# oleg-savchenko/jax_nbody_emulator_with_dj

Measured on AMD Instinct MI355X. Metric: voxels/sec (disp+vel) on 512^3 box, ndiv=4, higher is better.
Workload: dtype f32-equivalent: f16x3 split MFMA (3 f16 MFMAs per product, f32 accumulate)

## Files before the change

jax_nbody_emulator_with_dj_amd/csrc/nbe_kernels_h3.hip:

```cpp

#include "nbe_kernels_internal.h"
#include <cstdlib>
#include <cstdio>
#include <algorithm>

#ifndef NBE_DBG
#define NBE_DBG 0
#endif

namespace nbe {

extern __shared__ __attribute__((aligned(16))) f32x4 lds_h3[];

__device__ __forceinline__ void split4(const f32x4 v, half4& hi, half4& lo) {
#pragma unroll
    for (int e = 0; e < 4; ++e) {
        hi[e] = (_Float16)v[e];
        lo[e] = (_Float16)__builtin_fmaf((float)hi[e], -H3_SCALE, v[e] * H3_SCALE);
    }
}
__device__ __forceinline__ f32x4 join4(const half4 hi, const half4 lo) {
    f32x4 v;
#pragma unroll
    for (int e = 0; e < 4; ++e) v[e] = (float)hi[e] + (float)lo[e] * H3_INV;
    return v;
}

template <bool VEL, bool SPLIT>
__device__ __forceinline__ void h3_store2(const ConvKArgs& a, int ct, int it, int lh, const long (&o)[2],
                                          const bool (&ok)[2], const f32x16 (&ym)[2], const f32x16 (&yc)[2],
                                          const f32x16 (&dm)[2], const f32x16 (&dc)[2]) {
    constexpr int PARTS = SPLIT ? 2 : 1;
    const bool act = a.flags & F_ACT, res = a.flags & F_RES;
    int unit[4];
    bool uok[4];
    f32x4 bv[4], gv[4];
    const bool gauge = VEL && a.gout;
#pragma unroll
    for (int k = 0; k < 4; ++k) {
        unit[k] = ct * 8 + 4 * it + k;
        uok[k] = unit[k] < a.cout_groups;
        if (!uok[k]) unit[k] = a.cout_groups - 1;
        bv[k] = *(const f32x4*)(a.bias + unit[k] * 8 + 4 * lh);
        if (gauge) gv[k] = *(const f32x4*)(a.gout + unit[k] * 8 + 4 * lh);
    }
    half4 rh[8], rl[8], dh[8], dl[8];
    if (res) {
#pragma unroll
        for (int p = 0; p < 8; ++p) {
            const long rb = ((long)(PARTS * unit[p & 3]) * a.res_pstride + o[p >> 2]) * 16 + 8 * lh;
            const long rlo = rb + a.res_pstride * 16;
            rh[p] = *(const half4*)((const char*)a.r + rb);
            if (SPLIT) rl[p] = *(const half4*)((const char*)a.r + rlo);
            if (VEL) {
                dh[p] = *(const half4*)((const char*)a.dr + rb);
                if (SPLIT) dl[p] = *(const half4*)((const char*)a.dr + rlo);
            }
        }
    }
#pragma unroll
    for (int p = 0; p < 8; ++p) {
        const int jt = p >> 2, k = p & 3;
        f32x4 v, dv;
#pragma unroll
        for (int e = 0; e < 4; ++e) {
            v[e] = ym[jt][4 * k + e] + (SPLIT ? yc[jt][4 * k + e] * H3_INV : 0.f) + bv[k][e];
            dv[e] = dm[jt][4 * k + e] + (SPLIT ? dc[jt][4 * k + e] * H3_INV : 0.f);
        }
        if (res) {
            if (SPLIT) {
                v += join4(rh[p], rl[p]);
                if (VEL) dv += join4(dh[p], dl[p]);
            } else {
#pragma unroll
                for (int e = 0; e < 4; ++e) {
                    v[e] += (float)rh[p][e];
                    if (VEL) dv[e] += (float)dh[p][e];
                }
            }
        }
        if (act) {
#pragma unroll
            for (int e = 0; e < 4; ++e) {
                if (VEL) dv[e] = v[e] > 0.f ? dv[e] : 0.01f * dv[e];
                v[e] = v[e] >= 0.f ? v[e] : 0.01f * v[e];
            }
        }
        if (gauge) {
#pragma unroll
            for (int e = 0; e < 4; ++e) dv[e] += gv[k][e] * v[e];
        }
        if (uok[k] && ok[jt]) {
            const long ob = ((long)(a.out_g0 + PARTS * unit[k]) * a.out_pstride + o[jt]) * 16 + 8 * lh;
            const long ol = ob + a.out_pstride * 16;
            half4 hi, lo;
            split4(v, hi, lo);
            *(half4*)((char*)a.y + ob) = hi;
            if (SPLIT) *(half4*)((char*)a.y + ol) = lo;
            if (VEL) {
                split4(dv, hi, lo);
                *(half4*)((char*)a.dy + ob) = hi;
                if (SPLIT) *(half4*)((char*)a.dy + ol) = lo;
            }
        }
    }
}


template <int MODE, bool SPLIT>
struct H3Geom {
    static constexpr int PARTS = SPLIT ? 2 : 1, UN = 2 * PARTS;
    static_assert(MODE != MODE_FLAT3, "3x3x3 layers run on the patch kernels");
    static constexpr int XV = 256;
    static constexpr int WP = UN * 64;
    static constexpr int XP = UN * XV;
};

template <int MODE, bool VEL, bool HAS_DX, bool SPLIT>
__global__ __launch_bounds__(512, 2) void conv_h3_kernel(ConvKArgs a) {
    typedef H3Geom<MODE, SPLIT> G;
    constexpr int XV = G::XV, WP = G::WP, XP = G::XP, PARTS = G::PARTS, UN = G::UN;
    constexpr bool DX = VEL && HAS_DX;
    constexpr int WB = WP * (VEL ? 2 : 1);
    constexpr int XB = XP * (DX ? 2 : 1);
    constexpr int OFF_DW = WP, OFF_DXX = XP;
    constexpr int XRING = 2 * WB;
    constexpr int NW_TOT = WB / 64, NX_TOT = (XB + 63) / 64;
    constexpr int NWS = (NW_TOT + 7) / 8, NXS = (NX_TOT + 7) / 8;
    static_assert(WB % 64 == 0, "weight stage must be whole wave-instructions");
    static_assert(XP % 32 == 0, "activation planes must be half-wave multiples");
    static_assert(NWS + NXS <= 9, "more DMA slots per wave than MFMA pairs in one stage");

    f32x4* lds = lds_h3;
    const int tid = threadIdx.x;
    const int lane = tid & 63;
    const int wave = __builtin_amdgcn_readfirstlane(tid >> 6);
    const int li = lane & 31, lh = lane >> 5;
    const int it = wave & 1, jq = wave >> 1;

    const int tile = xcd_tile(blockIdx.x, a.ntiles);
    const int ct = blockIdx.y;
    const long q0 = (long)tile * TILE_VOX;
    const int nstage = mode_nseg(MODE) * a.nchunk;
    const long HW = (long)a.H * a.W;

    int* inbase = (int*)(lds + XRING + 2 * XB);
    if (MODE == MODE_DOWN) {
        if (tid < TILE_VOX) {
            long o = q0 + tid;
            if (o > a.Q - 1) o = a.Q - 1;
            const int hw = a.Hv * a.Wv;
            const int zo = (int)(o / hw), rem = (int)(o - (long)zo * hw);
            const int yo = rem / a.Wv, xo = rem - yo * a.Wv;
            inbase[tid] = (int)((2L * zo * a.H + 2 * yo) * a.W + 2 * xo);
        }
        __syncthreads();
    }

    const char* wsrc[NWS];
    int wdst[NWS];
    const char* xsrc[NXS];
    int xdst[NXS];
#pragma unroll
    for (int t = 0; t < NWS; ++t) {
        const int n = wave + 8 * t;
        wsrc[t] = nullptr; wdst[t] = 0;
        if (n < NW_TOT) {
            const bool d = VEL && n >= WP / 64;
            const int m = n - (d ? WP / 64 : 0);
            wsrc[t] = (const char*)(d ? a.dw : a.w) + ((long)ct * nstage * WP + m * 64 + lane) * 16;
            wdst[t] = (d ? OFF_DW : 0) + m * 64;
        }
    }
#pragma unroll
    for (int t = 0; t < NXS; ++t) {
        const int n = wave + 8 * t;
        xsrc[t] = nullptr; xdst[t] = 0;
        if (n < NX_TOT) {
            const int u = n * 64 + lane;
            const bool tang = DX && u >= XP;
            const int uu = u - (tang ? XP : 0);
            const int pl = uu / XV, vl = uu - pl * XV;
            long v;
            if (MODE == MODE_DOWN) v = (long)inbase[vl];
            else v = q0 + a.in_off + vl;
            xsrc[t] = (const char*)(tang ? a.dx : a.x) + ((long)pl * a.in_pstride + v) * 16;
            xdst[t] = (tang ? OFF_DXX : 0) + uu;
            xdst[t] = __builtin_amdgcn_readfirstlane(xdst[t]);
        }
    }

    auto seg_offset = [&](int s) -> long {
        const int chunk = s / mode_nseg(MODE), seg = s - chunk * mode_nseg(MODE);
        long segoff;
        if (MODE == MODE_DOWN) segoff = (seg >> 2) * HW + ((seg >> 1) & 1) * a.W + (seg & 1);
        else segoff = 0;
        return ((long)chunk * UN * a.in_pstride + segoff) * 16;
    };
    auto dma_w = [&](int t, int s) {
        if (wave + 8 * t < NW_TOT) dma16((const float*)(wsrc[t] + (long)s * WP * 16), lds + (s & 1) * WB + wdst[t]);
    };
    auto dma_x = [&](int t, long xoff, int ring) {
        if (wave + 8 * t < NX_TOT) dma16((const float*)(xsrc[t] + xoff), lds + XRING + ring * XB + xdst[t]);
    };
    auto wait_all = [&]() { asm volatile("s_waitcnt vmcnt(0)" ::: "memory"); };
    auto barrier = [&]() { asm volatile("s_waitcnt lgkmcnt(0)\n\ts_barrier" ::: "memory"); };

    f32x16 ym[2], yc[2], dm[2], dc[2];
#pragma unroll
    for (int jt = 0; jt < 2; ++jt)
#pragma unroll
        for (int e = 0; e < 16; ++e) { ym[jt][e] = 0.f; yc[jt][e] = 0.f; dm[jt][e] = 0.f; dc[jt][e] = 0.f; }

    struct Ops { half8 wh, wl, dwh, dwl, xh[2], xl[2], dxh[2], dxl[2]; };
    auto load_ops = [&](const half8* wb, const half8* xb, Ops& o) {
        const int wo = (PARTS * lh) * 64 + 32 * it + li;
        o.wh = wb[wo];
        if (SPLIT) o.wl = wb[wo + 64];
        if (VEL) { o.dwh = wb[OFF_DW + wo]; if (SPLIT) o.dwl = wb[OFF_DW + wo + 64]; }
#pragma unroll
        for (int jt = 0; jt < 2; ++jt) {
            const int xo = (PARTS * lh) * XV + jq * 64 + 32 * jt + li;
            o.xh[jt] = xb[xo];
            if (SPLIT) o.xl[jt] = xb[xo + XV];
            if (DX) { o.dxh[jt] = xb[OFF_DXX + xo]; if (SPLIT) o.dxl[jt] = xb[OFF_DXX + xo + XV]; }
        }
    };
    auto mfma1 = [&](const Ops& o, int i) {
        const int jt = i / 9, k = i % 9;
        if (k == 0) ym[jt] = __builtin_amdgcn_mfma_f32_32x32x16_f16(o.wh, o.xh[jt], ym[jt], 0, 0, 0);
        if (SPLIT && k == 1) yc[jt] = __builtin_amdgcn_mfma_f32_32x32x16_f16(o.wh, o.xl[jt], yc[jt], 0, 0, 0);
        if (SPLIT && k == 2) yc[jt] = __builtin_amdgcn_mfma_f32_32x32x16_f16(o.wl, o.xh[jt], yc[jt], 0, 0, 0);
        if (VEL) {
            if (k == 3) dm[jt] = __builtin_amdgcn_mfma_f32_32x32x16_f16(o.dwh, o.xh[jt], dm[jt], 0, 0, 0);
            if (SPLIT && k == 4) dc[jt] = __builtin_amdgcn_mfma_f32_32x32x16_f16(o.dwh, o.xl[jt], dc[jt], 0, 0, 0);
            if (SPLIT && k == 5) dc[jt] = __builtin_amdgcn_mfma_f32_32x32x16_f16(o.dwl, o.xh[jt], dc[jt], 0, 0, 0);
        }
        if (DX) {
            if (k == 6) dm[jt] = __builtin_amdgcn_mfma_f32_32x32x16_f16(o.wh, o.dxh[jt], dm[jt], 0, 0, 0);
            if (SPLIT && k == 7) dc[jt] = __builtin_amdgcn_mfma_f32_32x32x16_f16(o.wh, o.dxl[jt], dc[jt], 0, 0, 0);
            if (SPLIT && k == 8) dc[jt] = __builtin_amdgcn_mfma_f32_32x32x16_f16(o.wl, o.dxh[jt], dc[jt], 0, 0, 0);
        }
    };

    {
        const long x0 = seg_offset(0);
#pragma unroll
        for (int t = 0; t < NXS; ++t) dma_x(t, x0, 0);
#pragma unroll
        for (int t = 0; t < NWS; ++t) dma_w(t, 0);
        wait_all();
        barrier();
    }

    int ring = 0;
    for (int s = 0; s < nstage; ++s) {
        const bool pw = s + 1 < nstage, px = s + 1 < nstage;
        const long xoff2 = px ? seg_offset(s + 1) : 0;
        const int ring2 = ring ^ 1;
        const half8* wb = (const half8*)(lds + (s & 1) * WB);
        const half8* xb = (const half8*)(lds + XRING + ring * XB);
        Ops o0, o1;
        load_ops(wb, xb, o0);
        __builtin_amdgcn_sched_barrier(0);
#pragma unroll
        for (int i = 0; i < 18; ++i) {
            mfma1(o0, i);
            if (i & 1) {
                const int t = i >> 1;
                if (t < NWS) { if (pw) dma_w(t, s + 1); }
                else if (t - NWS < NXS) { if (px) dma_x(t - NWS, xoff2, ring2); }
                __builtin_amdgcn_sched_barrier(0);
            }
        }
        __builtin_amdgcn_sched_barrier(0);
        __builtin_amdgcn_sched_barrier(0);
        wait_all();
        barrier();
        ring = ring == 1 ? 0 : ring + 1;
    }

    long o[2];
    bool ok[2];
#pragma unroll
    for (int jt = 0; jt < 2; ++jt) {
        const long q = q0 + jq * 64 + 32 * jt + li;
        ok[jt] = q < a.Q;
        if (MODE == MODE_DOWN) {
            o[jt] = q;
        } else {
            const int z = (int)(q / HW), rem = (int)(q - (long)z * HW);
            const int yy = rem / a.W, xx = rem - yy * a.W;
            ok[jt] = ok[jt] && xx < a.Wv && yy < a.Hv && z < a.Dv;
            o[jt] = ((long)(z * a.osz + a.oz) * a.Ho + (yy * a.osz + a.oy)) * a.Wo + (xx * a.osz + a.ox);
        }
        if (!ok[jt]) o[jt] = 0;
    }
    h3_store2<VEL, SPLIT>(a, ct, it, lh, o, ok, ym, yc, dm, dc);
}

constexpr int UP_XV = 256;
constexpr int UP_MAXCH = 4;
template <bool SPLIT> struct UpGeom {
    static constexpr int UN = SPLIT ? 4 : 2;
    static constexpr int XC = 2 * UN * UP_XV;
    static constexpr int WS = 2 * 2 * UN * 64;
    static constexpr int WBASE = UP_MAXCH * XC;
    static constexpr int LDS_UNITS = WBASE + 2 * WS;
};

template <bool SPLIT, bool VEL = true>
__global__ __launch_bounds__(512, 2) void up_h3_kernel(ConvKArgs a) {
    constexpr int UN = UpGeom<SPLIT>::UN, UP_XC = UpGeom<SPLIT>::XC, UP_WS = UpGeom<SPLIT>::WS, UP_WBASE = UpGeom<SPLIT>::WBASE;
    constexpr int PS = SPLIT ? 2 : 1;
    f32x4* lds = lds_h3;
    const half8* L8 = (const half8*)lds_h3;
    const int tid = threadIdx.x;
    const int lane = tid & 63;
    const int wave = __builtin_amdgcn_readfirstlane(tid >> 6);
    const int li = lane & 31, lh = lane >> 5;
    const int it = wave & 1, jq = wave >> 1;
    const int tile = xcd_tile(blockIdx.x, a.ntiles);
    const int ct = blockIdx.y;
    const long q0 = (long)tile * UP_XV;
    const int nchunk = a.nchunk, nstage = 2 * 4 * nchunk;
    const long HW = (long)a.H * a.W;

    for (int c = 0; c < nchunk; ++c) {
#pragma unroll
        for (int k = 0; k < (VEL ? UN : UN / 2); ++k) {
            const int n = wave + 8 * k;
            const int t = n / (4 * UN), u = (n >> 2) % UN, qd = n & 3;
            const long v = q0 + a.in_off + qd * 64 + lane;
            const char* src = (const char*)(t ? a.dx : a.x) + (((long)c * UN + u) * a.in_pstride + v) * 16;
            dma16((const float*)src, lds + c * UP_XC + (t * UN + u) * UP_XV + qd * 64);
        }
    }
    auto dma_w = [&](int st) {
        const int c = st % nchunk, pp = (st / nchunk) & 3;
#pragma unroll
        for (int k = 0; k < UN / 2; ++k) {
            const int n = wave + 8 * k;
            const int par = n / (2 * UN), d = (n / UN) & 1, m = n % UN;
            if (!VEL && d) continue;
            const char* src = (const char*)(d ? a.dw : a.w) + (long)(2 * pp + par) * a.set_stride +
                              (((long)ct * nchunk + c) * (UN * 64) + m * 64 + lane) * 16;
            dma16((const float*)src, lds + UP_WBASE + (st & 1) * UP_WS + n * 64);
        }
    };
    dma_w(0);
    asm volatile("s_waitcnt vmcnt(0)" ::: "memory");
    __syncthreads();

    f32x16 ym[2], yc[2], dm[2], dc[2];
    auto zero_acc = [&]() {
#pragma unroll
        for (int jt = 0; jt < 2; ++jt)
#pragma unroll
            for (int e = 0; e < 16; ++e) { ym[jt][e] = 0.f; yc[jt][e] = 0.f; dm[jt][e] = 0.f; dc[jt][e] = 0.f; }
    };
    zero_acc();

    for (int st = 0; st < nstage; ++st) {
        const int c = st % nchunk, pp = (st / nchunk) & 3, half = st / (4 * nchunk);
        if (st + 1 < nstage) dma_w(st + 1);
        const half8* wb = L8 + UP_WBASE + (st & 1) * UP_WS;
        const half8* xb = L8 + c * UP_XC;
        const int xo = (PS * lh) * UP_XV + half * 128 + jq * 32 + li;
        const half8 xh = xb[xo];
        half8 dxh = xh, xl = xh, dxl = xh;
        if (VEL) dxh = xb[UN * UP_XV + xo];
        if (SPLIT) { xl = xb[xo + UP_XV]; if (VEL) dxl = xb[UN * UP_XV + xo + UP_XV]; }
#pragma unroll
        for (int jt = 0; jt < 2; ++jt) {
            const int wo = jt * (2 * UN * 64) + (PS * lh) * 64 + 32 * it + li;
            const half8 wh = wb[wo];
            half8 dwh = wh;
            if (VEL) dwh = wb[UN * 64 + wo];
            if (!SPLIT) {
                ym[jt] = __builtin_amdgcn_mfma_f32_32x32x16_f16(wh, xh, ym[jt], 0, 0, 0);
                if (VEL) {
                    dm[jt] = __builtin_amdgcn_mfma_f32_32x32x16_f16(dwh, xh, dm[jt], 0, 0, 0);
                    dm[jt] = __builtin_amdgcn_mfma_f32_32x32x16_f16(wh, dxh, dm[jt], 0, 0, 0);
                }
                continue;
            }
            const half8 wl = wb[wo + 64];
            ym[jt] = __builtin_amdgcn_mfma_f32_32x32x16_f16(wh, xh, ym[jt], 0, 0, 0);
            yc[jt] = __builtin_amdgcn_mfma_f32_32x32x16_f16(wh, xl, yc[jt], 0, 0, 0);
            yc[jt] = __builtin_amdgcn_mfma_f32_32x32x16_f16(wl, xh, yc[jt], 0, 0, 0);
            if (!VEL) continue;
            const half8 dwl = wb[UN * 64 + wo + 64];
            dm[jt] = __builtin_amdgcn_mfma_f32_32x32x16_f16(dwh, xh, dm[jt], 0, 0, 0);
            dc[jt] = __builtin_amdgcn_mfma_f32_32x32x16_f16(dwh, xl, dc[jt], 0, 0, 0);
            dc[jt] = __builtin_amdgcn_mfma_f32_32x32x16_f16(dwl, xh, dc[jt], 0, 0, 0);
            dm[jt] = __builtin_amdgcn_mfma_f32_32x32x16_f16(wh, dxh, dm[jt], 0, 0, 0);
            dc[jt] = __builtin_amdgcn_mfma_f32_32x32x16_f16(wh, dxl, dc[jt], 0, 0, 0);
            dc[jt] = __builtin_amdgcn_mfma_f32_32x32x16_f16(wl, dxh, dc[jt], 0, 0, 0);
        }
        const bool epi = c == nchunk - 1;
        if (epi) {
            asm volatile("s_waitcnt vmcnt(0)" ::: "memory");
            const long q = q0 + half * 128 + jq * 32 + li;
            const int z = (int)(q / HW), rem = (int)(q - (long)z * HW);
            const int yy = rem / a.W, xx = rem - yy * a.W;
            const bool okq = q < a.Q && xx < a.Wv && yy < a.Hv && z < a.Dv;
            const long o0 = okq ? ((long)(2 * z + (pp >> 1)) * a.Ho + (2 * yy + (pp & 1))) * a.Wo + 2 * xx : 0;
            const long o[2] = {o0, o0 + (okq ? 1 : 0)};
            const bool ok[2] = {okq, okq};
            h3_store2<VEL, SPLIT>(a, ct, it, lh, o, ok, ym, yc, dm, dc);
            zero_acc();
            asm volatile("s_waitcnt lgkmcnt(0)\n\ts_barrier" ::: "memory");
        } else {
            asm volatile("s_waitcnt vmcnt(0) lgkmcnt(0)" ::: "memory");
            __syncthreads();
        }
    }
}

template <bool SPLIT, bool VEL = true>
static int launch_up_h3(ConvKArgs ka, int ctiles, hipStream_t s) {
    constexpr size_t smem = (size_t)UpGeom<SPLIT>::LDS_UNITS * 16;
    static_assert(smem <= 160 * 1024, "LDS budget of one CU");
    if (ka.nchunk > UP_MAXCH) return 1;
    ensure_lds_limit((const void*)up_h3_kernel<SPLIT, VEL>, smem);
    dim3 grid(ka.ntiles, ctiles, 1), block(512, 1, 1);
    hipLaunchKernelGGL((up_h3_kernel<SPLIT, VEL>), grid, block, smem, s, ka);
    return 0;
}

constexpr int HP_ROWS = 8, HP_COLS = 32;
constexpr int HP_RS = HP_COLS + 2;
constexpr int HP_PL = (HP_ROWS + 2) * HP_RS;

template <bool VEL, bool HAS_DX, bool SPLIT>
__global__ __launch_bounds__(512, 2) void conv_h3p_kernel(ConvKArgs a) {
    constexpr bool DX = VEL && HAS_DX;
    constexpr int PARTS = SPLIT ? 2 : 1, UN = 2 * PARTS;
    constexpr int HP_XP = UN * HP_PL;
    constexpr int HP_XPP = (HP_XP + 63) / 64 * 64;
    constexpr int WP = 3 * UN * 64;
    constexpr int WB = WP * (VEL ? 2 : 1);
    constexpr int XB = HP_XPP * (DX ? 2 : 1);
    constexpr int OFF_DW = WP, OFF_DXX = HP_XPP;
    constexpr int XBASE = 2 * WB;
    constexpr int NW_TOT = WB / 64, NX_TOT = XB / 64;
    constexpr int NWS = (NW_TOT + 7) / 8;
    constexpr int XPARTS = 3;
    constexpr int NXS = (NX_TOT + 8 * XPARTS - 1) / (8 * XPARTS);
    static_assert(NWS + NXS <= 9 && NXS <= 4, "DMA slots per wave");

    f32x4* lds = lds_h3;
    const int tid = threadIdx.x;
    const int lane = tid & 63;
    const int wave = __builtin_amdgcn_readfirstlane(tid >> 6);
    const int li = lane & 31, lh = lane >> 5;
    const int it = wave & 1, jq = wave >> 1;

    const int tile = xcd_tile(blockIdx.x, a.ntiles);
    const int ct = blockIdx.y;
    const int z = tile % a.Dv, tyx = tile / a.Dv;
    const int ty = tyx / a.tnx, tx = tyx - ty * a.tnx;
    const int y0 = ty * HP_ROWS, x0 = tx * HP_COLS;
    const int nstage = 9 * a.nchunk;

    const char* wsrc[NWS];
    int wdst[NWS];
    const char* xsrc[XPARTS][NXS];
    int xdst[XPARTS][NXS];
    int kx[XPARTS];
#pragma unroll
    for (int t = 0; t < NWS; ++t) {
        const int n = wave + 8 * t;
        wsrc[t] = nullptr; wdst[t] = 0;
        if (n < NW_TOT) {
            const bool d = VEL && n >= WP / 64;
            const int m = n - (d ? WP / 64 : 0);
            wsrc[t] = (const char*)(d ? a.dw : a.w) + ((long)ct * nstage * WP + m * 64 + lane) * 16;
            wdst[t] = (d ? OFF_DW : 0) + m * 64;
        }
    }
#pragma unroll
    for (int p = 0; p < XPARTS; ++p) {
        kx[p] = 0;
#pragma unroll
        for (int t = 0; t < NXS; ++t) {
            const int n = (p * NXS + t) * 8 + wave;
            xsrc[p][t] = nullptr; xdst[p][t] = 0;
            if (n < NX_TOT) {
                ++kx[p];
                const int u = n * 64 + lane;
                const bool tang = DX && u >= HP_XPP;
                int uu = u - (tang ? HP_XPP : 0);
                const int ud = uu;
                if (uu >= HP_XP) uu = HP_XP - 1;
                const int pl = uu / HP_PL, rem = uu - pl * HP_PL;
                const int row = rem / HP_RS, col = rem - row * HP_RS;
                xsrc[p][t] = (const char*)(tang ? a.dx : a.x) + ((long)pl * a.in_pstride + (long)row * a.W + col) * 16;
                xdst[p][t] = __builtin_amdgcn_readfirstlane((tang ? OFF_DXX : 0) + ud);
            }
        }
    }
    auto patch_offset = [&](int g) -> long {
        const int chunk = g / 3, dz = g - chunk * 3;
        return ((long)chunk * UN * a.in_pstride + ((long)(z + dz) * a.H + y0) * a.W + x0) * 16;
    };
    auto dma_w = [&](int t, int s) {
        if (wave + 8 * t < NW_TOT) dma16((const float*)(wsrc[t] + (long)s * WP * 16), lds + (s & 1) * WB + wdst[t]);
    };
    auto dma_x = [&](int p, int t, long xoff, int xb) {
        if ((p * NXS + t) * 8 + wave < NX_TOT) dma16((const float*)(xsrc[p][t] + xoff), lds + XBASE + xb * XB + xdst[p][t]);
    };

    f32x16 ym[2], yc[2], dm[2], dc[2];
#pragma unroll
    for (int jt = 0; jt < 2; ++jt)
#pragma unroll
        for (int e = 0; e < 16; ++e) { ym[jt][e] = 0.f; yc[jt][e] = 0.f; dm[jt][e] = 0.f; dc[jt][e] = 0.f; }

    struct Ops { half8 wh, wl, dwh, dwl, xh[2], xl[2], dxh[2], dxl[2]; };
    auto load_ops = [&](const half8* wb, const half8* xb, int dy, int dx, Ops& o) {
        const int wo = (dx * UN + PARTS * lh) * 64 + 32 * it + li;
        o.wh = wb[wo];
        if (SPLIT) o.wl = wb[wo + 64];
        if (VEL) { o.dwh = wb[OFF_DW + wo]; if (SPLIT) o.dwl = wb[OFF_DW + wo + 64]; }
#pragma unroll
        for (int jt = 0; jt < 2; ++jt) {
            const int xo = (PARTS * lh) * HP_PL + (2 * jq + jt + dy) * HP_RS + li + dx;
            o.xh[jt] = xb[xo];
            if (SPLIT) o.xl[jt] = xb[xo + HP_PL];
            if (DX) { o.dxh[jt] = xb[OFF_DXX + xo]; if (SPLIT) o.dxl[jt] = xb[OFF_DXX + xo + HP_PL]; }
        }
    };
    auto mfma1 = [&](const Ops& o, int i) {
        const int jt = i / 9, k = i % 9;
        if (k == 0) ym[jt] = __builtin_amdgcn_mfma_f32_32x32x16_f16(o.wh, o.xh[jt], ym[jt], 0, 0, 0);
        if (SPLIT && k == 1) yc[jt] = __builtin_amdgcn_mfma_f32_32x32x16_f16(o.wh, o.xl[jt], yc[jt], 0, 0, 0);
        if (SPLIT && k == 2) yc[jt] = __builtin_amdgcn_mfma_f32_32x32x16_f16(o.wl, o.xh[jt], yc[jt], 0, 0, 0);
        if (VEL) {
            if (k == 3) dm[jt] = __builtin_amdgcn_mfma_f32_32x32x16_f16(o.dwh, o.xh[jt], dm[jt], 0, 0, 0);
            if (SPLIT && k == 4) dc[jt] = __builtin_amdgcn_mfma_f32_32x32x16_f16(o.dwh, o.xl[jt], dc[jt], 0, 0, 0);
            if (SPLIT && k == 5) dc[jt] = __builtin_amdgcn_mfma_f32_32x32x16_f16(o.dwl, o.xh[jt], dc[jt], 0, 0, 0);
        }
        if (DX) {
            if (k == 6) dm[jt] = __builtin_amdgcn_mfma_f32_32x32x16_f16(o.wh, o.dxh[jt], dm[jt], 0, 0, 0);
            if (SPLIT && k == 7) dc[jt] = __builtin_amdgcn_mfma_f32_32x32x16_f16(o.wh, o.dxl[jt], dc[jt], 0, 0, 0);
            if (SPLIT && k == 8) dc[jt] = __builtin_amdgcn_mfma_f32_32x32x16_f16(o.wl, o.dxh[jt], dc[jt], 0, 0, 0);
        }
    };
    auto mfma_ops = [&](const Ops& o) {
#pragma unroll
        for (int i = 0; i < 18; ++i) mfma1(o, i);
    };

    {
        const long x0off = patch_offset(0);
#pragma unroll
        for (int p = 0; p < XPARTS; ++p)
#pragma unroll
            for (int t = 0; t < NXS; ++t) dma_x(p, t, x0off, 0);
#pragma unroll
        for (int t = 0; t < NWS; ++t) dma_w(t, 0);
        __syncthreads();
    }

    int g = 0, dy = 0;
    for (int s = 0; s < nstage; ++s) {
        const bool pw = s + 1 < nstage, px = 3 * (g + 1) < nstage;
        const long xoff = px ? patch_offset(g + 1) : 0;
        const half8* wb = (const half8*)(lds + (s & 1) * WB);
        const half8* xb = (const half8*)(lds + XBASE + (g & 1) * XB);
        const int nb = (g + 1) & 1;
        Ops o0, o1;
        load_ops(wb, xb, dy, 0, o0);
        load_ops(wb, xb, dy, 1, o1);
        __builtin_amdgcn_sched_barrier(0);
#pragma unroll
        for (int i = 0; i < 18; ++i) {
            mfma1(o0, i);
            if (i & 1) {
                const int t = i >> 1;
                if (t < NWS) { if (pw) dma_w(t, s + 1); }
                else if (t - NWS < NXS) {
                    if (px) {
                        if (dy == 0) dma_x(0, t - NWS, xoff, nb);
                        else if (dy == 1) dma_x(1, t - NWS, xoff, nb);
                        else dma_x(2, t - NWS, xoff, nb);
                    }
                }
                __builtin_amdgcn_sched_barrier(0);
            }
        }
        __builtin_amdgcn_sched_barrier(0);
        load_ops(wb, xb, dy, 2, o0);
        __builtin_amdgcn_sched_barrier(0);
        mfma_ops(o1);
        __builtin_amdgcn_sched_barrier(0);
        mfma_ops(o0);
        __builtin_amdgcn_sched_barrier(0);
        __syncthreads();
        if (++dy == 3) { dy = 0; ++g; }
    }

    long o[2];
    bool ok[2];
#pragma unroll
    for (int jt = 0; jt < 2; ++jt) {
        const int yy = y0 + 2 * jq + jt, xx = x0 + li;
        ok[jt] = yy < a.Hv && xx < a.Wv;
        o[jt] = ok[jt] ? ((long)z * a.Ho + yy) * a.Wo + xx : (long)z * a.Ho * a.Wo;
    }
    h3_store2<VEL, SPLIT>(a, ct, it, lh, o, ok, ym, yc, dm, dc);
}

constexpr int HQ_TAPU = 4 * 64;
constexpr int HQ_WA = 5 * HQ_TAPU, HQ_WB = 4 * HQ_TAPU;
constexpr int HQ_OFF_B = 2 * HQ_WA;
constexpr int HQ_PP = (HP_PL + 7) / 8 * 8;
constexpr int HQ_XT = 4 * HQ_PP;
constexpr int HQ_XB = 2 * HQ_XT;
constexpr int HQ_XBASE = HQ_OFF_B + 2 * HQ_WB;
constexpr int HQ_LDS_UNITS = HQ_XBASE + 2 * HQ_XB;

__device__ __forceinline__ float acc_read(const float& acc) {
    float v;
    asm volatile("v_accvgpr_read_b32 %0, %1" : "=v"(v) : "a"(acc));
    return v;
}

__device__ __forceinline__ void dma16s(const char* ubase, unsigned voff, f32x4* dst_wave_base) {
    const unsigned long ub = (unsigned long)ubase;
    ubase = (const char*)(((unsigned long)(unsigned)__builtin_amdgcn_readfirstlane((int)(ub >> 32)) << 32) |
                          (unsigned long)(unsigned)__builtin_amdgcn_readfirstlane((int)(unsigned)ub));
    asm volatile("" : "+v"(voff));
    __builtin_amdgcn_global_load_lds((const NBE_GLB_AS void*)(ubase + voff), (NBE_LDS_AS void*)dst_wave_base, 16, 0, 0);
}

__device__ unsigned long long h3q_stamps[16];

void h3q_read_stamps(double* out, hipStream_t s) {
    unsigned long long h[16] = {0};
    (void)hipStreamSynchronize(s);
    (void)hipMemcpyFromSymbol(h, HIP_SYMBOL(h3q_stamps), sizeof h, 0, hipMemcpyDeviceToHost);
    for (int i = 0; i < 16; ++i) out[i] = (double)h[i];
    unsigned long long z[16] = {0};
    (void)hipMemcpyToSymbol(HIP_SYMBOL(h3q_stamps), z, sizeof z, 0, hipMemcpyHostToDevice);
}

__global__ __launch_bounds__(512, 2) void conv_h3q_kernel(ConvKArgs a) {
#if NBE_DBG
    unsigned long long tk0 = __builtin_amdgcn_s_memtime(), tk[8] = {0, 0, 0, 0, 0, 0, 0, 0};
#define NBE_STAMP(i) { const unsigned long long t_ = __builtin_amdgcn_s_memtime(); tk[i] += t_ - tk0; tk0 = t_; }
#define NBE_STAGE_END(i, keep) { NBE_STAMP(i) wait_keep(keep); NBE_STAMP(i + 1) \
                                 asm volatile("s_barrier" ::: "memory"); NBE_STAMP(i + 2) }
#else
#define NBE_STAMP(i)
#define NBE_STAGE_END(i, keep) { wait_keep(keep); asm volatile("s_barrier" ::: "memory"); }
#endif
    f32x4* lds = lds_h3;
    const half8* L8 = (const half8*)lds_h3;
    const int tid = threadIdx.x;
    const int lane = tid & 63;
    const int wave = __builtin_amdgcn_readfirstlane(tid >> 6);
    const int c = lane & 15, q = lane >> 4, kh = q & 1, ks = q >> 1;
    const int it = wave & 1, jq = wave >> 1;

    const int nct = (a.cout_groups + 7) / 8;
    const int vt = xcd_tile(blockIdx.x, a.ntiles * nct);
    const int tile = vt / nct, ct = vt - tile * nct;
    const int z = tile % a.Dv, tyx = tile / a.Dv;
    const int ty = tyx / a.tnx, tx = tyx - ty * a.tnx;
    const int y0 = ty * HP_ROWS, x0 = tx * HP_COLS;
    const int ngroups = 3 * a.nchunk;

    const unsigned lane16 = (unsigned)lane * 16u;
    const long wct = (long)ct * ngroups * 9 * HQ_TAPU;
    auto dma_w = [&](int g, int second, int t) {
        const int per = (second ? HQ_WB : HQ_WA) / 64;
        const int n = wave + 8 * t;
        if (n >= 2 * per) return;
        const int set = n >= per ? 1 : 0, m = n - set * per;
        const long src = wct + (long)g * 9 * HQ_TAPU + (second ? 5 * HQ_TAPU : 0) + m * 64;
        dma16s((const char*)(set ? a.dw : a.w) + src * 16, lane16,
               lds + (second ? HQ_OFF_B : 0) + set * (second ? HQ_WB : HQ_WA) + m * 64);
    };
    unsigned xoff[3];
    bool xval[3];
#pragma unroll
    for (int t = 0; t < 3; ++t) {
        const int k = (wave + 8 * t) % 6;
        const int u = k * 64 + lane;
        xval[t] = u < HP_PL;
        const int uu = xval[t] ? u : HP_PL - 1;
        const int row = uu / HP_RS, col = uu - row * HP_RS;
        xoff[t] = (unsigned)(row * a.W + col) * 16u;
    }
    auto patch_offset = [&](int g) -> long {
        const int chunk = g / 3, dz = g - chunk * 3;
        return ((long)chunk * 4 * a.in_pstride + ((long)(z + dz) * a.H + y0) * a.W + x0) * 16;
    };
    auto dma_x = [&](int tensor, int t, long xo, int buf) {
        const int n = wave + 8 * t, pl = n / 6, k = n - 6 * pl;
        if (xval[t])
            dma16s((const char*)(tensor ? a.dx : a.x) + xo + (long)pl * a.in_pstride * 16, xoff[t],
                   lds + HQ_XBASE + buf * HQ_XB + tensor * HQ_XT + pl * HQ_PP + k * 64);
    };
// ... 1318 lines not shown
```

Measured before the change: 97.63 million.

## Remap up-conv waves to cover all voxels per pass, skipping empty cout passes

```diff
diff --git a/jax_nbody_emulator_with_dj_amd/csrc/nbe_kernels_h3.hip b/jax_nbody_emulator_with_dj_amd/csrc/nbe_kernels_h3.hip
--- a/jax_nbody_emulator_with_dj_amd/csrc/nbe_kernels_h3.hip
+++ b/jax_nbody_emulator_with_dj_amd/csrc/nbe_kernels_h3.hip
@@ -301,10 +301,11 @@
 
 constexpr int UP_XV = 256;
 constexpr int UP_MAXCH = 4;
+constexpr int UP_CT = 32;
 template <bool SPLIT> struct UpGeom {
     static constexpr int UN = SPLIT ? 4 : 2;
     static constexpr int XC = 2 * UN * UP_XV;
-    static constexpr int WS = 2 * 2 * UN * 64;
+    static constexpr int WS = 2 * 2 * UN * UP_CT;
     static constexpr int WBASE = UP_MAXCH * XC;
     static constexpr int LDS_UNITS = WBASE + 2 * WS;
 };
@@ -319,11 +320,10 @@
     const int lane = tid & 63;
     const int wave = __builtin_amdgcn_readfirstlane(tid >> 6);
     const int li = lane & 31, lh = lane >> 5;
-    const int it = wave & 1, jq = wave >> 1;
     const int tile = xcd_tile(blockIdx.x, a.ntiles);
     const int ct = blockIdx.y;
     const long q0 = (long)tile * UP_XV;
-    const int nchunk = a.nchunk, nstage = 2 * 4 * nchunk;
+    const int nchunk = a.nchunk, npass = a.cout_groups - 8 * ct > 4 ? 2 : 1, nstage = npass * 4 * nchunk;
     const long HW = (long)a.H * a.W;
 
     for (int c = 0; c < nchunk; ++c) {
@@ -337,15 +337,15 @@
         }
     }
     auto dma_w = [&](int st) {
-        const int c = st % nchunk, pp = (st / nchunk) & 3;
-#pragma unroll
-        for (int k = 0; k < UN / 2; ++k) {
-            const int n = wave + 8 * k;
-            const int par = n / (2 * UN), d = (n / UN) & 1, m = n % UN;
-            if (!VEL && d) continue;
-            const char* src = (const char*)(d ? a.dw : a.w) + (long)(2 * pp + par) * a.set_stride +
-                              (((long)ct * nchunk + c) * (UN * 64) + m * 64 + lane) * 16;
-            dma16((const float*)src, lds + UP_WBASE + (st & 1) * UP_WS + n * 64);
+        const int c = st % nchunk, pp = (st / nchunk) & 3, it = st / (4 * nchunk);
+        if (wave < 2 * UN) {
+            const int r0 = 2 * wave;
+            const int par = r0 / (2 * UN), d = (r0 / UN) & 1, m = r0 % UN + lh;
+            if (VEL || !d) {
+                const char* src = (const char*)(d ? a.dw : a.w) + (long)(2 * pp + par) * a.set_stride +
+                                  (((long)ct * nchunk + c) * (UN * 64) + m * 64 + UP_CT * it + li) * 16;
+                dma16((const float*)src, lds + UP_WBASE + (st & 1) * UP_WS + wave * 64);
+            }
         }
     };
     dma_w(0);
@@ -362,21 +362,21 @@
     zero_acc();
 
     for (int st = 0; st < nstage; ++st) {
-        const int c = st % nchunk, pp = (st / nchunk) & 3, half = st / (4 * nchunk);
+        const int c = st % nchunk, pp = (st / nchunk) & 3, it = st / (4 * nchunk);
         if (st + 1 < nstage) dma_w(st + 1);
         const half8* wb = L8 + UP_WBASE + (st & 1) * UP_WS;
         const half8* xb = L8 + c * UP_XC;
-        const int xo = (PS * lh) * UP_XV + half * 128 + jq * 32 + li;
+        const int xo = (PS * lh) * UP_XV + wave * 32 + li;
         const half8 xh = xb[xo];
         half8 dxh = xh, xl = xh, dxl = xh;
         if (VEL) dxh = xb[UN * UP_XV + xo];
         if (SPLIT) { xl = xb[xo + UP_XV]; if (VEL) dxl = xb[UN * UP_XV + xo + UP_XV]; }
 #pragma unroll
         for (int jt = 0; jt < 2; ++jt) {
-            const int wo = jt * (2 * UN * 64) + (PS * lh) * 64 + 32 * it + li;
+            const int wo = jt * (2 * UN * UP_CT) + (PS * lh) * UP_CT + li;
             const half8 wh = wb[wo];
             half8 dwh = wh;
-            if (VEL) dwh = wb[UN * 64 + wo];
+            if (VEL) dwh = wb[UN * UP_CT + wo];
             if (!SPLIT) {
                 ym[jt] = __builtin_amdgcn_mfma_f32_32x32x16_f16(wh, xh, ym[jt], 0, 0, 0);
                 if (VEL) {
@@ -385,12 +385,12 @@
                 }
                 continue;
             }
-            const half8 wl = wb[wo + 64];
+            const half8 wl = wb[wo + UP_CT];
             ym[jt] = __builtin_amdgcn_mfma_f32_32x32x16_f16(wh, xh, ym[jt], 0, 0, 0);
             yc[jt] = __builtin_amdgcn_mfma_f32_32x32x16_f16(wh, xl, yc[jt], 0, 0, 0);
             yc[jt] = __builtin_amdgcn_mfma_f32_32x32x16_f16(wl, xh, yc[jt], 0, 0, 0);
             if (!VEL) continue;
-            const half8 dwl = wb[UN * 64 + wo + 64];
+            const half8 dwl = wb[UN * UP_CT + wo + UP_CT];
             dm[jt] = __builtin_amdgcn_mfma_f32_32x32x16_f16(dwh, xh, dm[jt], 0, 0, 0);
             dc[jt] = __builtin_amdgcn_mfma_f32_32x32x16_f16(dwh, xl, dc[jt], 0, 0, 0);
             dc[jt] = __builtin_amdgcn_mfma_f32_32x32x16_f16(dwl, xh, dc[jt], 0, 0, 0);
@@ -401,7 +401,7 @@
         const bool epi = c == nchunk - 1;
         if (epi) {
             asm volatile("s_waitcnt vmcnt(0)" ::: "memory");
-            const long q = q0 + half * 128 + jq * 32 + li;
+            const long q = q0 + wave * 32 + li;
             const int z = (int)(q / HW), rem = (int)(q - (long)z * HW);
             const int yy = rem / a.W, xx = rem - yy * a.W;
             const bool okq = q < a.Q && xx < a.Wv && yy < a.Hv && z < a.Dv;
```

Result: no change. 97.77 million, median of 2 (+0.1%).
